# cvg/GeoCalib

Hardware: AMD Instinct MI355X
Metric: images/sec LM calibration (640x480, 20 iters) (higher is better)
Workload: dtype f32

## Files before the change

### geocalib_amd/csrc/gclm_api.hip

```cpp
#include <chrono>
#include <cstdarg>
#include <cstdio>
#include <cstdlib>
#include <cstring>
#include <new>
#include <string>
#include <thread>
#include <vector>

#include "gclm_args.h"
#include "gclm_internal.h"

using namespace gclm;

#ifndef GCLM_FUSED_MAX_WORKGROUPS
#define GCLM_FUSED_MAX_WORKGROUPS 768
#endif
#ifndef GCLM_ROW_PAIRS_DEFAULT
#define GCLM_ROW_PAIRS_DEFAULT -1
#endif
#ifndef GCLM_CONF_PACK_MIN_PIXELS
#define GCLM_CONF_PACK_MIN_PIXELS (256ll << 20)
#endif
#ifndef GCLM_ISO_FINAL
// ... 228 lines not shown
    geo = plan_geometry(B, H, W, aligned16, h->sweep_iters, c.camera_model);
    const bool few = (long long)B * geo.nchunks <= GCLM_FUSED_MAX_WORKGROUPS;
    const bool fusable = !c.shared_intrinsics && geo.vec == 4 && (B == 1 || !c.early_stop) && B > 0 &&
                         !(c.early_stop && h->stop_comm);
    const bool pairable = geo.vec == 4 && five && !(H & 1) && H >= 4 &&
                          (h->row_pairs > 0 ? sweep_has_mirror(c.camera_model) : sweep_mirror_builtin(c.camera_model));
    bool pairs = false;
    if (pairable && h->row_pairs < 0) {
        pairs = !few;
    } else if (pairable && h->row_pairs > 0) {
        pairs = !(h->fused_mode == 1 && fusable);
    }
    one_launch = !pairs && fusable && (h->fused_mode == 1 || (h->fused_mode < 0 && few));
    if (pairs) geo = plan_geometry(B, H, W, aligned16, h->sweep_iters, c.camera_model, true);
}

bool wants_conf_pack(const gclm_handle* h, const Plan& p, bool five, int sweeps, long long pixels) {
    const int model = h->cfg.camera_model;
    return model == GCLM_PINHOLE && p.geo.vec == 4 && five && !p.one_launch && sweeps >= 2 && h->conf_pack != 0 &&
           sweep_has_conf_pack(model) && (h->conf_pack > 0 || (pixels >= GCLM_CONF_PACK_MIN_PIXELS && sweeps >= 6));
}

int make_plan(gclm_handle* h, Plan& p, const Fields& f, int B, int H, int W, const float* sin_lat, int sweeps,
              bool may_pack = true) {
    const int Bp = B > 0 ? B : 1, model = h->cfg.camera_model;
    p = Plan{};
    p.f = f;
    p.choose_walk(h, Bp, H, W, f.aligned16(), f.five());
    SolveCtx& c = h->ctx;
    c.cfg = h->cfg;
    c.B = B; c.H = H; c.W = W; c.nchunks = p.geo.nchunks;
    const bool float4_five = p.geo.vec == 4 && f.five();
    if (sin_lat && float4_five && is_aligned(sin_lat, 16) && (p.one_launch || model != GCLM_PINHOLE)) p.given = sin_lat;
    const bool keep = !p.given && h->slat_plane != 0 && !p.one_launch && float4_five && sweeps >= 2 &&
                      !(h->slat_plane < 0 && model == GCLM_PINHOLE) && sweep_has_slat_plane(model);
    if (int rc = ensure_workspace(h, Bp, p.geo.nchunks, c.n_groups)) return rc;
    p.slat = static_cast<float*>(ensure_plane(h, h->slat, keep ? (size_t)B * H * W * sizeof(float) : 0));
    const long long pixels = (long long)B * H * W;
    const bool pack = may_pack && !p.given && !p.slat && wants_conf_pack(h, p, f.five(), sweeps, pixels);
    p.cpack = static_cast<uint32_t*>(ensure_plane(h, h->cpack, pack ? (size_t)pixels * sizeof(uint32_t) : 0));
    h->cpack_images = p.cpack ? B : 0;
    h->sh.active = false;
    return 0;
}

SweepArgs Plan::next_sweep(const gclm_handle* h, const PBlock* pb, bool loop_params, int stop_step) {
    SweepArgs a{};
    a.up = f.up; a.lat = f.lat; a.upc = f.up ? f.upc : nullptr; a.latc = f.latc;
    a.pb = pb; a.ctrl = h->ctx.ctrl; a.partials = h->ctx.partials;
    a.B = h->ctx.B; a.H = h->ctx.H; a.W = h->ctx.W;
    a.nchunks = geo.nchunks; a.vec = geo.vec;
    a.wu = geo.wu; a.cu = geo.cu; a.nstrips = geo.nstrips; a.rpi = geo.rpi; a.rows_per_block = geo.rows_per_block; a.wpt = geo.wpt; a.jobs = geo.jobs;
    a.hrows = geo.hrows; a.mirror = geo.mirror;
    a.log_focal = loop_params ? h->cfg.use_log_focal : h->ctx.iso_final;
    a.stop_step = stop_step;
    a.up_scale = h->cfg.up_loss_fn_scale; a.lat_scale = h->cfg.lat_loss_fn_scale;
    if (given) {
        a.slat = const_cast<float*>(given);
        a.lat = given;
        a.slat_mode = 2;
    } else if (slat) {
        a.slat = slat;
        if (slat_filled) a.lat = slat;
        a.slat_mode = slat_filled ? 2 : 1;
        slat_filled = true;
    }
    if (cpack) {
        a.cpack = cpack;
        a.cpack_flags = h->ctx.cpack_flags;
        a.cpack_mode = cpack_filled ? 2 : 1;
        cpack_filled = true;
    }
    return a;
}

struct Pacer {
    gclm_handle* h;
    bool paced;
    bool waiting;
    bool stop_seen = false;

    Pacer(gclm_handle* handle, bool single_image_early_stop)
        : h(handle), paced(handle->paced_depth > 0 && single_image_early_stop && handle->progress_host) {
        if (paced && h->paced_cooldown > 0) { --h->paced_cooldown; paced = false; }
        if (paced) h->epoch = (h->epoch + 1) & kPacedEpochMask;
        waiting = paced;
    }
    bool reported(int launch) {
        const unsigned v = __atomic_load_n(h->progress_host, __ATOMIC_ACQUIRE);
        if (((v >> kPacedEpochShift) & kPacedEpochMask) != h->epoch) return false;
        if (v & kPacedStopBit) stop_seen = true;
        return stop_seen || (v & 0xffffu) >= (unsigned)(launch + 1);
    }
    void wait_before(int step) {
        if (!waiting || step < h->paced_depth) return;
        const auto t0 = std::chrono::steady_clock::now();
        for (unsigned spin = 0; !reported(step - h->paced_depth); ++spin) {
            if (spin < 256) continue;
            std::this_thread::yield();
            if ((spin & 0xf) == 0 && std::chrono::steady_clock::now() - t0 > std::chrono::microseconds(kPacedPatienceUs)) {
                waiting = false;
                h->paced_cooldown = kPacedCooldown;
                break;
            }
        }
    }
};

int solve_empty_shard(gclm_handle* h, int H, int W, const InitArgs& ia, hipStream_t s) {
// ... 76 lines not shown
    if (int rc = make_plan(h, p, f, B, H, W, d_sin_lat, h->cfg.num_steps + 1)) return rc;
    if (d_record) {
        p.one_launch = false;
        GCLM_HIP(h, hipMemsetAsync(d_record, 0, sizeof(float) * GCLM_LM_RECORD_STRIDE * (size_t)B * h->cfg.num_steps, s));
        return solve_two_launches_per_step(h, p, ia, d_cam_out, d_grav_out, d_info_out, s, d_record);
    }
    if (p.one_launch) return solve_one_launch_per_step(h, p, ia, d_cam_out, d_grav_out, d_info_out, s);
    return solve_two_launches_per_step(h, p, ia, d_cam_out, d_grav_out, d_info_out, s);
}

}

namespace gclm {
Geometry plan_geometry(int B, int H, int W, bool aligned16, int sweep_iters, int camera_model, bool mirror) {
    Geometry g;
    g.vec = (aligned16 && (W % 4 == 0)) ? 4 : 1;
    g.mirror = (mirror && g.vec == 4 && H % 2 == 0 && H >= 4) ? 1 : 0;
    g.hrows = g.mirror ? H / 2 : H;
    const int rows = g.hrows;
    g.wu = W / g.vec;
    auto waste = [](int used, int lanes) { return (int)(50.0 * (lanes - used) / lanes); };
    if (g.wu <= kMaxTile) {
        g.nstrips = 1;
        g.cu = g.wu;
        g.rpi = 1;
        int best = 1 << 30;
        for (int r = 1; r * g.wu <= kMaxTile; ++r) {
            const int lanes = (r * g.wu + 63) / 64 * 64;
            const int score = waste(r * g.wu, lanes) * 1024 + lanes / 64;
            if (score < best) { best = score; g.rpi = r; }
        }
        g.wpt = (g.rpi * g.wu + 63) / 64;
    } else {
        g.rpi = 1;
        g.cu = 256;
        int best = 1 << 30;
        for (int cu = 128; cu <= kMaxTile; cu += 64) {
            const int ns = (g.wu + cu - 1) / cu;
            const int score = waste(g.wu, ns * cu) * 1024 + cu / 64;
            if (score < best) { best = score; g.cu = cu; }
        }
        g.nstrips = (g.wu + g.cu - 1) / g.cu;
        g.wpt = g.cu / 64;
    }
    int builtin = g.mirror ? 10 : 20;
    if (camera_model != GCLM_PINHOLE && rows % (g.rpi * (g.mirror ? 15 : 30)) == 0) builtin = g.mirror ? 15 : 30;
    int iters = (sweep_iters >= 1 && sweep_iters <= 4096) ? sweep_iters : builtin;
    auto jobs = [&](int it) { return g.nstrips * g.wpt * ((rows + g.rpi * it - 1) / (g.rpi * it)); };
    auto chunks = [&](int it) { return (jobs(it) + kBlock / 64 - 1) / (kBlock / 64); };
    while (iters > 2 && (long long)B * chunks(iters) < 2048) iters = iters > 5 ? iters / 2 : iters - 1;
    g.rows_per_block = g.rpi * iters;
    g.jobs = jobs(iters);
    g.nchunks = chunks(iters);
    return g;
}
}

extern "C" {

int gclm_version(void) { return GCLM_VERSION; }

int gclm_abi_config_size(void) { return (int)sizeof(gclm_config); }

int gclm_default_config(gclm_config* cfg) {
    if (!cfg) return -1;
    std::memset(cfg, 0, sizeof(*cfg));
    cfg->struct_size = (int32_t)sizeof(gclm_config);
    cfg->abi_version = GCLM_VERSION;
    cfg->device = 0;
    cfg->camera_model = GCLM_PINHOLE;
    cfg->num_steps = 30;
    cfg->lambda0 = 0.1f;
    cfg->early_stop = 1;
    cfg->atol = 1e-8f;
    cfg->rtol = 1e-8f;
    cfg->use_spherical_manifold = 1;
    cfg->use_log_focal = 1;
    cfg->up_loss_fn_scale = 1e-2f;
    cfg->lat_loss_fn_scale = 1e-2f;
    cfg->estimate_gravity = cfg->estimate_focal = cfg->estimate_dist = 1;
    cfg->compute_uncertainty = 1;
    return 0;
}

int gclm_create(gclm_handle** out, const gclm_config* cfg) {
    if (!out || !cfg) return fail(nullptr, -1, "gclm_create: null argument");
    *out = nullptr;
    char abuf[256];
    if (const char* msg = abi_mismatch(cfg, abuf)) return fail(nullptr, -5, "gclm_create: %s", msg);
    if (const char* msg = validate(*cfg)) return fail(nullptr, -2, "gclm_create: %s", msg);
    const int device = cfg->device;
    int ndev = 0;
    if (hipGetDeviceCount(&ndev) != hipSuccess || ndev <= 0)
        return fail(nullptr, -11, "gclm_create: no HIP device visible (the HIP path has no CPU fallback)");
    if (device < 0 || device >= ndev) return fail(nullptr, -2, "gclm_create: device %d out of range (%d devices)", device, ndev);
    gclm_handle* h = new (std::nothrow) gclm_handle();
    if (!h) return fail(nullptr, -12, "gclm_create: out of host memory");
    h->cfg = *cfg;
    h->device = device;
    *out = h;
    return 0;
}

int gclm_configure(gclm_handle* h, const gclm_config* cfg) {
    if (!h || !cfg) return -1;
    char abuf[256];
// ... 375 lines not shown
```

### geocalib_amd/csrc/gclm_internal.h

```cpp
#pragma once
#include <hip/hip_runtime.h>
#include <stdint.h>

#include <type_traits>

#include "../../include/gclm.h"

namespace gclm {

constexpr int kBlock = 256;
constexpr int kMaxTile = 512;
constexpr int kNAcc = 16;
constexpr int kNAccMax = 24;
constexpr int kPBlockFloats = 20;
constexpr int kMaxP = GCLM_MAX_PARAMS;
constexpr int kStateFloats = 16;
constexpr int kMaxCallImages = 65535;

enum Acc { A_CU = 0, A_CL = 1, A_G0 = 2, A_H00 = 6 };
__host__ __device__ constexpr int acc_pm(int camera_model) { return camera_model == GCLM_RADIAL ? 5 : 4; }
__host__ __device__ constexpr int acc_floats(int camera_model) { return camera_model == GCLM_RADIAL ? kNAccMax : kNAcc; }
__host__ __device__ constexpr int acc_h(int pm, int i, int j) {
    return 2 + pm + i * pm - (i * (i - 1)) / 2 + (j - i);
}
__host__ __device__ constexpr int num_dist_params(int camera_model) {
    return camera_model == GCLM_PINHOLE ? 0 : (camera_model == GCLM_RADIAL ? 2 : 1);
}

template <typename F>
hipError_t with_camera_model(int camera_model, F&& f) {
    switch (camera_model) {
        case GCLM_PINHOLE: return f(std::integral_constant<int, GCLM_PINHOLE>{});
        case GCLM_SIMPLE_RADIAL: return f(std::integral_constant<int, GCLM_SIMPLE_RADIAL>{});
        case GCLM_RADIAL: return f(std::integral_constant<int, GCLM_RADIAL>{});
        case GCLM_SIMPLE_DIVISIONAL: return f(std::integral_constant<int, GCLM_SIMPLE_DIVISIONAL>{});
        default: return hipErrorInvalidValue;
    }
}

struct __attribute__((aligned(16))) PBlock {
    float ifx, ify, cx, cy;
    float ga, gb, gc, k1;
    float T00, T01, T10, T11;
    float T20, T21, wfx, wfy;
    float k2, pad0, pad1, pad2;
};
static_assert(sizeof(PBlock) == kPBlockFloats * 4, "PBlock layout");

struct __attribute__((aligned(16))) State {
    float w, h, fx, fy, cx, cy, k1, k2;
    float gx, gy, gz;
    float lambda, prev_cost, fails, init_cu, init_cl;
};
static_assert(sizeof(State) == kStateFloats * 4, "State layout");

struct Ctrl {
    int stopped;
    int final_sel;
    int pad[2];
    int notclose[GCLM_MAX_STEPS + 4];
};

__host__ __device__ inline bool stop_fired_before(const Ctrl* ctrl, int step) {
    return step >= 2 && ctrl->notclose[step - 1] == 0;
}

struct SweepArgs {
    const float* up;
    const float* lat;
    const float* upc;
    const float* latc;
    const PBlock* pb;
    const Ctrl* ctrl;
    float* partials;
    int B, H, W;
    int nchunks;
    int vec;
    int wu, cu, nstrips;
    int rpi, rows_per_block;
    int wpt, jobs;
    int log_focal;
    int stop_step;
    float up_scale, lat_scale;
    float* slat;
    int slat_mode;
    int hrows;
    int mirror;
    uint32_t* cpack;
    unsigned* cpack_flags;
    int cpack_mode;
};

struct Geometry {
    int vec, nchunks;
    int wu, cu, nstrips, rpi, rows_per_block, wpt, jobs;
    int mirror, hrows;
};

struct SolveCtx {
    gclm_config cfg;
    int B, H, W, nchunks;
    int iso_final;
    int n_groups, group_size;
    const int32_t* group_of_frame;
    State* state[2];
    PBlock* pb[2];
    PBlock* pb_final;
    float* partials;
    float* partials2;
    float* frame_sys;
    Ctrl* ctrl;
    unsigned* cpack_flags;
};
struct InitArgs {
    const float* cam;
    const float* grav;
    const float* scales;
    const float* prior_focal;
    const float* prior_gravity;
    const float* prior_dist;
    int prior_dist_cols;
    const float* up;
    const float* lat;
};
struct FusedArgs {
    SolveCtx c;
    int step;
    int is_final;
    const float* partials_in;
    unsigned* progress;
    unsigned epoch;
    InitArgs ia;
    int init_here;
};
constexpr unsigned kPacedStopBit = 1u << 16;
constexpr unsigned kPacedEpochShift = 20, kPacedEpochMask = 0xfffu;
constexpr int kPacedPatienceUs = 2000;
constexpr int kPacedCooldown = 64;
constexpr int kMaxMergeParts = 8;
struct MergeStopArgs {
    const Ctrl* ctrl[kMaxMergeParts];
    float* info[kMaxMergeParts];
    int B[kMaxMergeParts];
    int n, num_steps;
};
constexpr int kMaxUpsampleTensors = 8;
struct UpsampleMulti {
    const float* src[kMaxUpsampleTensors];
    float* dst[kMaxUpsampleTensors];
// ... 108 lines not shown
```

### geocalib_amd/csrc/gclm_pass.hip

```cpp
#include <type_traits>

#include "gclm_internal.h"
#include "gclm_device.h"

#ifndef GCLM_MIN_WAVES
#define GCLM_MIN_WAVES 1
#endif
#ifndef GCLM_DIV_WAVES
#define GCLM_DIV_WAVES 3
#endif
#ifndef GCLM_PINHOLE_WAVES
#define GCLM_PINHOLE_WAVES 6
#endif
#ifndef GCLM_RADIAL_WAVES
#define GCLM_RADIAL_WAVES 3
#endif
#ifndef GCLM_REUSE_TNUV
#define GCLM_REUSE_TNUV 1
#endif
#ifndef GCLM_PINHOLE_LDS
#define GCLM_PINHOLE_LDS 51200
#endif
#ifndef GCLM_CPACK_LDS
#define GCLM_CPACK_LDS 30720
#endif
#ifndef GCLM_DYN_LDS
#define GCLM_DYN_LDS 0
#endif
#ifndef GCLM_LAT_PAIRS
#define GCLM_LAT_PAIRS 1
#endif
#ifndef GCLM_MIRROR_WAVES
#define GCLM_MIRROR_WAVES 2
#endif
#ifndef GCLM_MIRROR_WAVES_RADIAL
#define GCLM_MIRROR_WAVES_RADIAL 3
#endif

#ifndef GCLM_TRACE
#define GCLM_TRACE 0
#endif
#if GCLM_TRACE
__device__ unsigned long long g_gclm_trace[64][16];
#define GCLM_T(step, slot) do { if (threadIdx.x == 0 && blockIdx.x == GCLM_TRACE_WG && blockIdx.y == 0 && (step) < 64) g_gclm_trace[(step)][(slot)] = wall_clock64(); } while (0)
extern "C" int gclm_debug_trace(unsigned long long* out) {
    return hipMemcpyFromSymbol(out, HIP_SYMBOL(g_gclm_trace), sizeof(g_gclm_trace)) == hipSuccess ? 0 : -1;
}
#ifndef GCLM_TRACE_WG
#define GCLM_TRACE_WG 0
#endif
#else
#define GCLM_T(step, slot) do {} while (0)
#endif

namespace gclm {

namespace {

typedef float f2 __attribute__((ext_vector_type(2)));

__device__ __forceinline__ float vfma(float a, float b, float c) { return fmaf(a, b, c); }
__device__ __forceinline__ f2 vfma(f2 a, f2 b, f2 c) { return __builtin_elementwise_fma(a, b, c); }
__device__ __forceinline__ float vrsq(float a) { return __frsqrt_rn(a); }
__device__ __forceinline__ f2 vrsq(f2 a) { return f2{__frsqrt_rn(a.x), __frsqrt_rn(a.y)}; }
__device__ __forceinline__ float vrcp_hw(float a) { return __builtin_amdgcn_rcpf(a); }
__device__ __forceinline__ f2 vrcp_hw(f2 a) { return f2{__builtin_amdgcn_rcpf(a.x), __builtin_amdgcn_rcpf(a.y)}; }
__device__ __forceinline__ float vsqrt_hw(float a) { return __builtin_amdgcn_sqrtf(a); }
__device__ __forceinline__ f2 vsqrt_hw(f2 a) { return f2{__builtin_amdgcn_sqrtf(a.x), __builtin_amdgcn_sqrtf(a.y)}; }
__device__ __forceinline__ float vmax(float a, float b) { return fmaxf(a, b); }
__device__ __forceinline__ f2 vmax(f2 a, f2 b) { return f2{fmaxf(a.x, b.x), fmaxf(a.y, b.y)}; }
__device__ __forceinline__ float vclamp(float a, float lo, float hi) { return fminf(fmaxf(a, lo), hi); }
__device__ __forceinline__ f2 vclamp(f2 a, float lo, float hi) {
    return f2{fminf(fmaxf(a.x, lo), hi), fminf(fmaxf(a.y, lo), hi)};
}
__device__ __forceinline__ float vrsq_min1(float y) {
    return __builtin_amdgcn_fmed3f(__frsqrt_rn(y), 0.0f, 1.0f);
}
// ... 462 lines not shown
        }
    }
}

template <int MODEL, typename F>
__device__ __forceinline__ void lat_pair_accumulate(F (&acc)[Layout<MODEL>::NACC], const PixelShared<MODEL, F>& S, const LatRow<F>& A,
                                                    const LatRow<F>& B) {
    constexpr int PM = Layout<MODEL>::PM, ND = Layout<MODEL>::ND;
    const Radial<F>& R = S.R;
    F f[1 + ND];
    f[0] = -vfma(R.tau1x2, S.r2, R.tau);
#pragma unroll
    for (int j = 0; j < ND; ++j) f[1 + j] = R.dtau[j];
#pragma unroll
    for (int r = 0; r < 2; ++r) {
        const LatRow<F>& L = r == 0 ? A : B;
        const F w0 = L.wgt * L.l0, w1 = L.wgt * L.l1;
        acc[A_G0 + 0] = vfma(w0, L.rl, acc[A_G0 + 0]);
        acc[A_G0 + 1] = vfma(w1, L.rl, acc[A_G0 + 1]);
        acc[acc_h(PM, 0, 0)] = vfma(w0, L.l0, acc[acc_h(PM, 0, 0)]);
        acc[acc_h(PM, 0, 1)] = vfma(w0, L.l1, acc[acc_h(PM, 0, 1)]);
        acc[acc_h(PM, 1, 1)] = vfma(w1, L.l1, acc[acc_h(PM, 1, 1)]);
    }
    const F a1 = A.wgt * A.hu, a2 = B.wgt * B.hu;
    const F sAA = vfma(a2, B.hu, a1 * A.hu), sC = vfma(a2, B.rl, a1 * A.rl);
    const F sB0 = vfma(a2, B.l0, a1 * A.l0), sB1 = vfma(a2, B.l1, a1 * A.l1);
#pragma unroll
    for (int m = 0; m <= ND; ++m) {
        acc[A_G0 + 2 + m] = vfma(sC, f[m], acc[A_G0 + 2 + m]);
        acc[acc_h(PM, 0, 2 + m)] = vfma(sB0, f[m], acc[acc_h(PM, 0, 2 + m)]);
        acc[acc_h(PM, 1, 2 + m)] = vfma(sB1, f[m], acc[acc_h(PM, 1, 2 + m)]);
#pragma unroll
        for (int n = m; n <= ND; ++n) acc[acc_h(PM, 2 + m, 2 + n)] = vfma(sAA, f[m] * f[n], acc[acc_h(PM, 2 + m, 2 + n)]);
    }
}

template <int MODEL, bool HAS_UP, bool LOGF, typename F, int EMIT = 0, int GMODE = 0>
__device__ __forceinline__ void pixel_accumulate(const PBlock& P, const HuberK& hk, F u, F px, float v, F dux, F duy,
                                                 F slat, F cu, F cl, F (&acc)[Layout<MODEL>::NACC],
                                                 [[maybe_unused]] float* j_up = nullptr,
                                                 [[maybe_unused]] float* j_lat = nullptr,
                                                 [[maybe_unused]] bool patch = false) {
    PixelShared<MODEL, F> S;
    pixel_shared<MODEL, LOGF, F, GMODE>(P, u, v, patch, S);
    pixel_stage<MODEL, HAS_UP, LOGF, F, EMIT>(P, hk, S, u, px, v, dux, duy, slat, cu, cl, acc, j_up, j_lat);
}

constexpr int kWaveSumLane = 63;
template <int CTRL, int ROW_MASK>
__device__ __forceinline__ float dpp_add(float v) {
    const int moved = __builtin_amdgcn_update_dpp(0, __builtin_bit_cast(int, v), CTRL, ROW_MASK, 0xF, false);
    return v + __builtin_bit_cast(float, moved);
}
__device__ __forceinline__ float wave_sum(float v) {
    v = dpp_add<0xB1, 0xF>(v);
    v = dpp_add<0x4E, 0xF>(v);
    v = dpp_add<0x141, 0xF>(v);
    v = dpp_add<0x140, 0xF>(v);
    v = dpp_add<0x142, 0xA>(v);
    v = dpp_add<0x143, 0xC>(v);
    return v;
}

template <int VEC>
struct Lane;
template <>
struct Lane<4> {
    using F = f2;
    using V = float4;
    static constexpr int kPairs = 2;
    static __device__ __forceinline__ V ld(const float* base, uint32_t byte_off) {
        typedef float v4 __attribute__((ext_vector_type(4)));
        const v4* p = reinterpret_cast<const v4*>(reinterpret_cast<const char*>(base) + byte_off);
        const v4 t = __builtin_nontemporal_load(p);
        return make_float4(t.x, t.y, t.z, t.w);
    }
    static __device__ __forceinline__ void st(float* base, uint32_t byte_off, const F (&v)[2]) {
        typedef float v4 __attribute__((ext_vector_type(4)));
        __builtin_nontemporal_store(v4{v[0].x, v[0].y, v[1].x, v[1].y},
                                    reinterpret_cast<v4*>(reinterpret_cast<char*>(base) + byte_off));
    }
    typedef uint32_t P __attribute__((ext_vector_type(4)));
    static __device__ __forceinline__ P ldp(const uint32_t* base, uint32_t byte_off) {
        return __builtin_nontemporal_load(reinterpret_cast<const P*>(reinterpret_cast<const char*>(base) + byte_off));
    }
    static __device__ __forceinline__ void stp(uint32_t* base, uint32_t byte_off, P w) {
        __builtin_nontemporal_store(w, reinterpret_cast<P*>(reinterpret_cast<char*>(base) + byte_off));
    }
    static __device__ __forceinline__ F get(const V& v, int k) { return k == 0 ? f2{v.x, v.y} : f2{v.z, v.w}; }
    static __device__ __forceinline__ V ones() { return make_float4(1.f, 1.f, 1.f, 1.f); }
    static __device__ __forceinline__ bool any_zero(F a) { return a.x == 0.f || a.y == 0.f; }
    static __device__ __forceinline__ float max_of(const F (&t)[2]) { return fmaxf(fmaxf(fmaxf(t[0].x, t[0].y), t[1].x), t[1].y); }
    static __device__ __forceinline__ F fold(F a) { return f2{fold_halfpi(a.x), fold_halfpi(a.y)}; }
    static __device__ __forceinline__ F xcoord(int x, int k) {
        const float x0 = (float)(x + 2 * k);
        return f2{x0, x0 + 1.0f};
    }
};
template <>
struct Lane<1> {
    using F = float;
    using V = float;
    using P = uint32_t;
    static constexpr int kPairs = 1;
    static __device__ __forceinline__ V ld(const float* base, uint32_t byte_off) {
        return *reinterpret_cast<const float*>(reinterpret_cast<const char*>(base) + byte_off);
    }
    static __device__ __forceinline__ void st(float* base, uint32_t byte_off, const F (&v)[1]) {
        *reinterpret_cast<float*>(reinterpret_cast<char*>(base) + byte_off) = v[0];
    }
    static __device__ __forceinline__ F get(const V& v, int) { return v; }
    static __device__ __forceinline__ V ones() { return 1.f; }
    static __device__ __forceinline__ bool any_zero(F a) { return a == 0.f; }
    static __device__ __forceinline__ float max_of(const F (&t)[1]) { return t[0]; }
    static __device__ __forceinline__ F fold(F a) { return fold_halfpi(a); }
    static __device__ __forceinline__ F xcoord(int x, int) { return (float)x; }
};

template <int VEC>
struct LaneJob {
    bool live;
    int y, y_end, xu;
    uint32_t off, off_step;
};
template <int VEC>
__device__ __forceinline__ LaneJob<VEC> lane_job(const SweepArgs& a, const int chunk) {
    const int tid = threadIdx.x;
    const int lane = tid & 63, wave = tid >> 6;
    const int job = chunk * (kBlock / 64) + wave;
    const int tile = job / a.wpt, tw = job - tile * a.wpt;
    const int rowblock = tile / a.nstrips, strip = tile - rowblock * a.nstrips;
    const int f = tw * 64 + lane;
    const int tr = f / a.cu, tc = f - tr * a.cu;
    LaneJob<VEC> j;
    j.xu = strip * a.cu + tc;
    j.live = job < a.jobs && tr < a.rpi && j.xu < a.wu;
    j.y_end = min((rowblock + 1) * a.rows_per_block, a.hrows);
    j.y = rowblock * a.rows_per_block + tr;
    j.off = ((uint32_t)j.y * (uint32_t)a.W + (uint32_t)(j.xu * VEC)) * 4u;
    j.off_step = (uint32_t)a.rpi * (uint32_t)a.W * 4u;
    return j;
}

template <int VEC>
struct RowData {
    typename Lane<VEC>::V vux, vuy, vlat, vcu, vcl;
    typename Lane<VEC>::P vpk;
};
template <bool HAS_UP, bool HAS_UPC, bool HAS_LATC, int VEC, int CPACK = 0>
__device__ __forceinline__ RowData<VEC> load_row(const float* upx, const float* upy, const float* lat, const float* upc,
                                                 const float* latc, const uint32_t off,
                                                 [[maybe_unused]] const uint32_t* cpk = nullptr) {
    using L = Lane<VEC>;
    RowData<VEC> r;
    r.vcu = L::ones();
    r.vcl = L::ones();
    if constexpr (HAS_UP) {
        r.vux = L::ld(upx, off);
        r.vuy = L::ld(upy, off);
    }
    r.vlat = L::ld(lat, off);
    if constexpr (CPACK == 2) {
        r.vpk = L::ldp(cpk, off);
    } else {
        if constexpr (HAS_UP && HAS_UPC) r.vcu = L::ld(upc, off);
        if constexpr (HAS_LATC) r.vcl = L::ld(latc, off);
    }
    return r;
}

template <int VEC, int CPACK>
__device__ __forceinline__ void row_conf(const RowData<VEC>& r, typename Lane<VEC>::F (&cu)[Lane<VEC>::kPairs],
                                         typename Lane<VEC>::F (&cl)[Lane<VEC>::kPairs], [[maybe_unused]] uint32_t* cp_out,
                                         [[maybe_unused]] const uint32_t off, [[maybe_unused]] bool* cp_bad) {
    using L = Lane<VEC>;
    if constexpr (CPACK == 0) {
#pragma unroll
        for (int k = 0; k < L::kPairs; ++k) { cu[k] = L::get(r.vcu, k); cl[k] = L::get(r.vcl, k); }
    } else {
        static_assert(VEC == 4, "the packed confidence plane: float4 path only");
        auto decode2 = [](uint32_t qa, uint32_t qb) { return f2{(float)qa, (float)qb} * dev::kConfStep; };
        if constexpr (CPACK == 2) {
            const uint32_t w[4] = {r.vpk.x, r.vpk.y, r.vpk.z, r.vpk.w};
#pragma unroll
            for (int k = 0; k < 2; ++k) {
                cu[k] = decode2(w[2 * k] & 0xffffu, w[2 * k + 1] & 0xffffu);
// ... 97 lines not shown
    }
#endif
}

template <int MODEL, bool HAS_UP, bool LOGF, int VEC, int SLAT, bool SHARE>
__device__ __forceinline__ void row_math_mirror(const PBlock& P, const HuberK& hk, const typename Lane<VEC>::F (&col_u)[Lane<VEC>::kPairs],
                                                const typename Lane<VEC>::F (&col_px)[Lane<VEC>::kPairs], const int y, const int y2,
                                                const RowData<VEC>& r, const RowData<VEC>& rm,
                                                typename Lane<VEC>::F (&acc)[Layout<MODEL>::NACC], const bool col_zero,
                                                const bool div_k_tiny, float* slat_out, const uint32_t off, const uint32_t off2) {
    using L = Lane<VEC>;
    using F = typename L::F;
    F slat[L::kPairs], slat2[L::kPairs];
    row_slat<VEC, SLAT>(r, slat, slat_out, off);
    row_slat<VEC, SLAT>(rm, slat2, slat_out, off2);
    const float v = ((float)y - P.cy) * P.ify;
    const float v2 = SHARE ? -v : ((float)y2 - P.cy) * P.ify;
    constexpr int GM = MODEL == GCLM_SIMPLE_DIVISIONAL ? 1 : 0;
    const bool patch = div_k_tiny || __builtin_amdgcn_ballot_w64(col_zero && (v == 0.f || v2 == 0.f)) != 0;
#pragma unroll
    for (int k = 0; k < L::kPairs; ++k) {
        PixelShared<MODEL, F> S;
        pixel_shared<MODEL, LOGF, F, GM>(P, col_u[k], v, patch, S);
        if constexpr (SHARE && LOGF && GCLM_LAT_PAIRS) {
            pixel_stage<MODEL, HAS_UP, LOGF, F, 0, 1>(P, hk, S, col_u[k], col_px[k], v, L::get(r.vux, k), L::get(r.vuy, k), slat[k],
                                                      L::get(r.vcu, k), L::get(r.vcl, k), acc);
            pixel_stage<MODEL, HAS_UP, LOGF, F, 0, 1>(P, hk, S, col_u[k], col_px[k], v2, L::get(rm.vux, k), L::get(rm.vuy, k), slat2[k],
                                                      L::get(rm.vcu, k), L::get(rm.vcl, k), acc);
            LatRow<F> la, lb;
            pixel_stage<MODEL, HAS_UP, LOGF, F, 3, 2>(P, hk, S, col_u[k], col_px[k], v, L::get(r.vux, k), L::get(r.vuy, k), slat[k],
                                                      L::get(r.vcu, k), L::get(r.vcl, k), acc, nullptr, nullptr, &la);
            pixel_stage<MODEL, HAS_UP, LOGF, F, 3, 2>(P, hk, S, col_u[k], col_px[k], v2, L::get(rm.vux, k), L::get(rm.vuy, k), slat2[k],
                                                      L::get(rm.vcu, k), L::get(rm.vcl, k), acc, nullptr, nullptr, &lb);
            lat_pair_accumulate<MODEL, F>(acc, S, la, lb);
        } else {
        pixel_stage<MODEL, HAS_UP, LOGF, F>(P, hk, S, col_u[k], col_px[k], v, L::get(r.vux, k), L::get(r.vuy, k), slat[k],
                                            L::get(r.vcu, k), L::get(r.vcl, k), acc);
        if constexpr (!SHARE) pixel_shared<MODEL, LOGF, F, GM>(P, col_u[k], v2, patch, S);
        pixel_stage<MODEL, HAS_UP, LOGF, F>(P, hk, S, col_u[k], col_px[k], v2, L::get(rm.vux, k), L::get(rm.vuy, k), slat2[k],
                                            L::get(rm.vcu, k), L::get(rm.vcl, k), acc);
        }
    }
}

template <int MODEL, bool HAS_UP, bool HAS_UPC, bool HAS_LATC, bool LOGF, int VEC, int PRE = 0, int SLAT = 0, bool MIRROR = false,
          int CPACK = 0>
__device__ __forceinline__ void sweep_body(const SweepArgs& a, const PBlock& P, const int b, const int chunk,
                                           [[maybe_unused]] const LaneJob<VEC>* pj = nullptr,
                                           [[maybe_unused]] const RowData<VEC>* pre = nullptr) {
    constexpr int NACC = Layout<MODEL>::NACC;
    static_assert(PRE == 0 || SLAT != 1, "the prefetched iterations of the one-launch-per-step kernel store no plane");
    static_assert(CPACK == 0 || (PRE == 0 && !MIRROR && SLAT == 0 && VEC == 4 && HAS_UP && HAS_UPC && HAS_LATC),
                  "the packed confidence plane: the plain five-plane float4 sweep");
    const int tid = threadIdx.x;
    HuberK hk;
    hk.a2u = a.up_scale * a.up_scale;
    hk.inv_a2u = 1.0f / hk.a2u;
    hk.a2l = a.lat_scale * a.lat_scale;
    hk.inv_a2l = 1.0f / hk.a2l;

    const size_t N = (size_t)a.H * a.W;
    const float* upx = HAS_UP ? a.up + (size_t)b * 2 * N : nullptr;
    const float* upy = HAS_UP ? upx + N : nullptr;
    const float* lat = a.lat + (size_t)b * N;
    const float* upc = HAS_UPC ? a.upc + (size_t)b * N : nullptr;
    const float* latc = HAS_LATC ? a.latc + (size_t)b * N : nullptr;
    [[maybe_unused]] float* slat_out = SLAT == 1 ? a.slat + (size_t)b * N : nullptr;
    [[maybe_unused]] uint32_t* cpk = CPACK != 0 ? a.cpack + (size_t)b * N : nullptr;
    [[maybe_unused]] bool cp_bad = false;

    using L = Lane<VEC>;
    using F = typename L::F;
    F acc[NACC];
#pragma unroll
    for (int i = 0; i < NACC; ++i) acc[i] = F(0.f);

    const int lane = tid & 63, wave = tid >> 6;
    const LaneJob<VEC> j = PRE > 0 ? *pj : lane_job<VEC>(a, chunk);
    const int xu = j.xu;
    const bool live = j.live;
    const int y_end = j.y_end;
    int y = j.y;
    uint32_t off = j.off;
    const uint32_t off_step = j.off_step;
    F col_u[L::kPairs], col_px[L::kPairs];
#pragma unroll
    for (int k = 0; k < L::kPairs; ++k) {
        col_u[k] = (L::xcoord(xu * VEC, k) - P.cx) * P.ifx;
        col_px[k] = vfma(col_u[k], vsplat(col_u[k], -P.gc), vsplat(col_u[k], P.ga));
    }
    [[maybe_unused]] bool col_zero = false;
    [[maybe_unused]] const bool div_k_tiny = !(fabsf(P.k1) >= 1e-20f);
    if constexpr (MODEL == GCLM_SIMPLE_DIVISIONAL) {
#pragma unroll
        for (int k = 0; k < L::kPairs; ++k) col_zero = col_zero || L::any_zero(col_u[k]);
    }
    if (live) {
        if constexpr (PRE > 0) {
#pragma unroll
            for (int it = 0; it < PRE; ++it) {
                if (y < y_end) {
                    row_math<MODEL, HAS_UP, LOGF, VEC, SLAT>(P, hk, col_u, col_px, y, pre[it], acc, col_zero, div_k_tiny);
                    y += a.rpi;
                    off += off_step;
                }
            }
        }
        if constexpr (MIRROR) {
            static_assert(PRE == 0 && VEC == 4 && HAS_UP && HAS_UPC && HAS_LATC, "row pairs: five-plane float4 sweep");
            const bool centered = P.cy + P.cy == (float)a.H;
            const uint32_t row_bytes = (uint32_t)a.W * 4u, col_bytes = (uint32_t)(xu * VEC) * 4u;
            auto pair = [&](auto share) {
                const int y2 = y == 0 ? (a.H >> 1) : a.H - y;
                const uint32_t off2 = (uint32_t)y2 * row_bytes + col_bytes;
                const RowData<VEC> r = load_row<HAS_UP, HAS_UPC, HAS_LATC, VEC>(upx, upy, lat, upc, latc, off);
                const RowData<VEC> rm = load_row<HAS_UP, HAS_UPC, HAS_LATC, VEC>(upx, upy, lat, upc, latc, off2);
                __builtin_amdgcn_sched_barrier(0);
                row_math_mirror<MODEL, HAS_UP, LOGF, VEC, SLAT, decltype(share)::value>(P, hk, col_u, col_px, y, y2, r, rm, acc, col_zero,
                                                                                    div_k_tiny, slat_out, off, off2);
                y += a.rpi;
                off += off_step;
            };
            if (centered) {
                if (__builtin_amdgcn_ballot_w64(y == 0) != 0 && y < y_end) pair(std::false_type{});
                while (y < y_end) pair(std::true_type{});
            } else {
                while (y < y_end) pair(std::false_type{});
            }
        } else
        for (; y < y_end; y += a.rpi, off += off_step) {
            const RowData<VEC> r = load_row<HAS_UP, HAS_UPC, HAS_LATC, VEC, CPACK>(upx, upy, lat, upc, latc, off, cpk);
            __builtin_amdgcn_sched_barrier(0);
            row_math<MODEL, HAS_UP, LOGF, VEC, SLAT, CPACK>(P, hk, col_u, col_px, y, r, acc, col_zero, div_k_tiny, slat_out, off,
                                                            cpk, &cp_bad);
        }
        if constexpr (CPACK == 1) { if (cp_bad) atomicOr(a.cpack_flags + b, 1u); }
    }

    __shared__ float red[kBlock / 64][NACC];
    float wsum[NACC];
#pragma unroll
    for (int i = 0; i < NACC; ++i) wsum[i] = wave_sum(hsum(acc[i]));
    if (lane == kWaveSumLane) {
#pragma unroll
        for (int i = 0; i < NACC; ++i) red[wave][i] = wsum[i];
    }
    __syncthreads();
    if (tid < NACC) {
        float s = 0.f;
#pragma unroll
        for (int w = 0; w < kBlock / 64; ++w) s += red[w][tid];
        if (tid == A_CU) s *= hk.a2u;
        if (tid == A_CL) s *= hk.a2l;
        a.partials[((size_t)b * a.nchunks + chunk) * NACC + tid] = s;
    }
}

template <int MODEL, bool HAS_UP, bool HAS_UPC, bool HAS_LATC, bool LOGF, int VEC, int SLAT = 0, bool MIRROR = false>
__global__ __launch_bounds__(kBlock, MIRROR ? (MODEL == GCLM_RADIAL && LOGF ? GCLM_MIRROR_WAVES_RADIAL : GCLM_MIRROR_WAVES) : (VEC == 4 && MODEL == GCLM_RADIAL) ? GCLM_RADIAL_WAVES : (VEC == 4 && MODEL > GCLM_RADIAL) ? GCLM_DIV_WAVES : (VEC == 4 && MODEL == GCLM_SIMPLE_RADIAL) ? 4 : (VEC == 4 && MODEL == GCLM_PINHOLE && LOGF) ? (SLAT == 0 ? GCLM_PINHOLE_WAVES : 5) : GCLM_MIN_WAVES) void sweep_kernel(
    const SweepArgs a) {
    if (stop_fired_before(a.ctrl, a.stop_step)) return;
    const int b = blockIdx.y, chunk = blockIdx.x;
    const PBlock P = a.pb[b];
    sweep_body<MODEL, HAS_UP, HAS_UPC, HAS_LATC, LOGF, VEC, 0, SLAT, MIRROR>(a, P, b, chunk);
}

template <bool LOGF, int CPACK>
__global__ __launch_bounds__(kBlock, 5) void conf_pack_sweep_kernel(const SweepArgs a) {
    if (stop_fired_before(a.ctrl, a.stop_step)) return;
    const int b = blockIdx.y, chunk = blockIdx.x;
    const PBlock P = a.pb[b];
    if constexpr (CPACK == 2) {
        if (a.cpack_flags[b] != 0) {
            sweep_body<GCLM_PINHOLE, true, true, true, LOGF, 4, 0, 0, false, 0>(a, P, b, chunk);
            return;
        }
    }
    sweep_body<GCLM_PINHOLE, true, true, true, LOGF, 4, 0, 0, false, CPACK>(a, P, b, chunk);
}

template <int MODEL, bool HAS_UP, bool HAS_UPC, bool HAS_LATC, bool LOGF, int SLAT = 0>
__global__ __launch_bounds__(kBlock) void fused_step_kernel(const SweepArgs a, const FusedArgs f) {
    using namespace dev;
    constexpr int PM = Layout<MODEL>::PM, NACC = Layout<MODEL>::NACC;
    const SolveCtx& c = f.c;
    const gclm_config& cfg = c.cfg;
    static_assert(SLAT == 0 || (SLAT == 2 && HAS_UP && HAS_UPC && HAS_LATC), "a handed plane: five-plane launches only");
    const int b = blockIdx.y, chunk = blockIdx.x, step = f.step;
    GCLM_T(step, 0);
    __shared__ PBlock Ps;
    __shared__ int go;
    int stop_j = 0;
    if (cfg.early_stop) {
        if (!f.is_final) {
            if (step >= 3 && c.ctrl->notclose[step - 2] == 0) return;
        } else {
            const int lane = threadIdx.x & 63;
            for (int j0 = 1; j0 <= step - 2 && stop_j == 0; j0 += 64) {
                const int j = j0 + lane;
                const int v = j <= step - 2 ? c.ctrl->notclose[j] : 1;
                const unsigned long long m = __builtin_amdgcn_ballot_w64(v == 0);
                if (m) stop_j = j0 + __builtin_ctzll(m);
            }
        }
    }
    constexpr int kFusedPre = 2;
    const LaneJob<4> pj = lane_job<4>(a, chunk);
    RowData<4> pre[kFusedPre];
    auto request_fields = [&]() {
        const size_t N = (size_t)a.H * a.W;
        const float* upx = HAS_UP ? a.up + (size_t)b * 2 * N : nullptr;
        const float* upy = HAS_UP ? upx + N : nullptr;
// ... 209 lines not shown
    if (weight) weight[i] = isx * c;
    if (second) second[i] = y <= 1.0f ? 0.f : -isx / (2.0f * y * a2);
}

constexpr bool sweep_exists(int model, bool up, bool upc, bool latc, bool logf, int vec, int slat, bool mirror, int cpack = 0) {
    const bool five = up && upc && latc;
    if (model < GCLM_PINHOLE || model > GCLM_SIMPLE_DIVISIONAL || (upc && !up) || slat < 0 || slat > 2) return false;
    if (cpack != 0) return (cpack == 1 || cpack == 2) && model == GCLM_PINHOLE && five && vec == 4 && slat == 0 && !mirror;
    if (vec != 4) return vec == 1 && !logf && slat == 0 && !mirror;
    if (mirror) return five && (model == GCLM_RADIAL || model == GCLM_SIMPLE_DIVISIONAL);
    return slat == 0 || five;
}
constexpr bool fused_exists(int model, bool up, bool upc, bool latc, int slat) {
    if (model < GCLM_PINHOLE || model > GCLM_SIMPLE_DIVISIONAL || (upc && !up)) return false;
    return slat == 0 || (slat == 2 && up && upc && latc);
}
constexpr int kMirrorBuiltinModels = (1 << GCLM_RADIAL) | (1 << GCLM_SIMPLE_DIVISIONAL);

template <typename F>
hipError_t with_flags(F&& f) { return f(); }
template <typename F, typename... Bools>
hipError_t with_flags(F&& f, bool first, Bools... rest) {
    auto bind = [&](auto c) { return with_flags([&](auto... cs) { return f(c, cs...); }, rest...); };
    return first ? bind(std::true_type{}) : bind(std::false_type{});
}
template <typename F>
hipError_t with_slat_mode(int slat_mode, F&& f) {
    switch (slat_mode) {
        case 0: return f(std::integral_constant<int, 0>{});
        case 1: return f(std::integral_constant<int, 1>{});
        case 2: return f(std::integral_constant<int, 2>{});
        default: return hipErrorInvalidValue;
    }
}

}

hipError_t launch_sweep(int camera_model, const SweepArgs& a, hipStream_t s) {
    if (a.B <= 0) return hipSuccess;
    if ((a.slat_mode != 0 && a.slat == nullptr) || (a.mirror != 0 && ((a.H & 1) || a.hrows * 2 != a.H))) return hipErrorInvalidValue;
    if (a.cpack_mode != 0 && (a.cpack == nullptr || a.cpack_flags == nullptr)) return hipErrorInvalidValue;
    const dim3 grid(a.nchunks, a.B), block(kBlock);
    const bool up = a.up != nullptr, vec4 = a.vec == 4;
    return with_camera_model(camera_model, [&](auto m) {
        return with_slat_mode(a.slat_mode, [&](auto sl) {
          return with_slat_mode(a.cpack_mode, [&](auto cp) {
            return with_flags([&](auto u, auto uc, auto lc, auto lf, auto v4, auto mir) {
                constexpr int MODEL = decltype(m)::value, SLAT = decltype(sl)::value, VEC = decltype(v4)::value ? 4 : 1;
                constexpr int CPACK = decltype(cp)::value;
                constexpr bool U = decltype(u)::value, UC = decltype(uc)::value, LC = decltype(lc)::value,
                               LOGF = decltype(lf)::value, MIRROR = decltype(mir)::value;
                if constexpr (sweep_exists(MODEL, U, UC, LC, LOGF, VEC, SLAT, MIRROR, CPACK)) {
                    constexpr unsigned lds = (MODEL == GCLM_PINHOLE && VEC == 4 && SLAT == 0 && !MIRROR && GCLM_DYN_LDS == 0)
                                                 ? (CPACK == 2 ? GCLM_CPACK_LDS : GCLM_PINHOLE_LDS) : GCLM_DYN_LDS;
                    if constexpr (CPACK != 0) hipLaunchKernelGGL((conf_pack_sweep_kernel<LOGF, CPACK>), grid, block, lds, s, a);
                    else hipLaunchKernelGGL((sweep_kernel<MODEL, U, UC, LC, LOGF, VEC, SLAT, MIRROR>), grid, block, lds, s, a);
                    return hipGetLastError();
                } else {
                    return hipErrorInvalidValue;
                }
            }, up, up && a.upc != nullptr, a.latc != nullptr, vec4 && a.log_focal != 0, vec4, a.mirror != 0);
          });
        });
    });
}

bool sweep_has_mirror(int camera_model) { return sweep_exists(camera_model, true, true, true, true, 4, 0, true); }
bool sweep_mirror_builtin(int camera_model) { return sweep_has_mirror(camera_model) && ((kMirrorBuiltinModels >> camera_model) & 1) != 0; }
bool sweep_has_slat_plane(int camera_model) { return sweep_exists(camera_model, true, true, true, true, 4, 1, false); }
bool sweep_has_conf_pack(int camera_model) { return sweep_exists(camera_model, true, true, true, true, 4, 0, false, 1); }

hipError_t launch_fused_step(int camera_model, const SweepArgs& a, const FusedArgs& f, hipStream_t s) {
    if (a.B <= 0) return hipSuccess;
    if (a.vec != 4 || (a.slat_mode != 0 && (a.slat == nullptr || a.lat != a.slat))) return hipErrorInvalidValue;
    const dim3 grid(a.nchunks, a.B), block(kBlock);
    const bool up = a.up != nullptr;
    return with_camera_model(camera_model, [&](auto m) {
        return with_slat_mode(a.slat_mode, [&](auto sl) {
            return with_flags([&](auto u, auto uc, auto lc, auto lf) {
                constexpr int MODEL = decltype(m)::value, SLAT = decltype(sl)::value;
                constexpr bool U = decltype(u)::value, UC = decltype(uc)::value, LC = decltype(lc)::value, LOGF = decltype(lf)::value;
                if constexpr (fused_exists(MODEL, U, UC, LC, SLAT)) {
                    hipLaunchKernelGGL((fused_step_kernel<MODEL, U, UC, LC, LOGF, SLAT>), grid, block, 0, s, a, f);
                    return hipGetLastError();
                } else {
                    return hipErrorInvalidValue;
                }
            }, up, up && a.upc != nullptr, a.latc != nullptr, a.log_focal != 0);
        });
    });
}

hipError_t launch_residual_fields(int camera_model, const float* d_up, const float* d_lat, const float* d_cam,
                                  const float* d_grav, int B, int H, int W, float* d_r_up, float* d_r_lat, hipStream_t s) {
    if (B <= 0 || H <= 0 || W <= 0) return hipSuccess;
    const dim3 grid((unsigned)(((size_t)H * W + kBlock - 1) / kBlock), B), block(kBlock);
    return with_camera_model(camera_model, [&](auto m) {
        hipLaunchKernelGGL(residual_kernel<decltype(m)::value>, grid, block, 0, s, d_up, d_lat, d_cam, d_grav, H, W, d_r_up, d_r_lat);
        return hipGetLastError();
    });
}

hipError_t launch_huber_costs(const float* d_residual, size_t n, int dim, float scale, const float* d_conf,
                              float* d_cost, float* d_weight, float* d_second, hipStream_t s) {
    if (n == 0) return hipSuccess;
    hipLaunchKernelGGL(huber_costs_kernel, dim3((unsigned)((n + 255) / 256)), dim3(256), 0, s, d_residual, n, dim, scale,
                       d_conf, d_cost, d_weight, d_second);
// ... 16 lines not shown
```

Before: 58920.

## Precompute divisors and Huber constants on host, batch DPP wave reductions

Replaces the integer divisions in lane job mapping with host-precomputed magic-multiply reciprocals, and passes the Huber scale constants in the kernel arguments instead of recomputing them per thread. It also makes the wave index scalar via readfirstlane, reduces only the live accumulators with row-broadcast DPP steps batched eight at a time in inline asm, and changes the LDS and launch-bounds settings for some variants. The goal is fewer VALU instructions in setup and the reduction epilogue, at the cost of hand-written asm hazards (s_nop) and subtle range limits on the fast division.

Measured after the change: 59140 (median of 6 runs). Within noise of the previous version (+0.4%).

```diff
diff --git a/geocalib_amd/csrc/gclm_api.hip b/geocalib_amd/csrc/gclm_api.hip
--- a/geocalib_amd/csrc/gclm_api.hip
+++ b/geocalib_amd/csrc/gclm_api.hip
@@ -304,9 +304,12 @@
     a.nchunks = geo.nchunks; a.vec = geo.vec;
     a.wu = geo.wu; a.cu = geo.cu; a.nstrips = geo.nstrips; a.rpi = geo.rpi; a.rows_per_block = geo.rows_per_block; a.wpt = geo.wpt; a.jobs = geo.jobs;
     a.hrows = geo.hrows; a.mirror = geo.mirror;
+    a.div_wpt = geo.div_wpt; a.div_nstrips = geo.div_nstrips; a.div_cu = geo.div_cu;
     a.log_focal = loop_params ? h->cfg.use_log_focal : h->ctx.iso_final;
     a.stop_step = stop_step;
     a.up_scale = h->cfg.up_loss_fn_scale; a.lat_scale = h->cfg.lat_loss_fn_scale;
+    a.a2u = a.up_scale * a.up_scale; a.inv_a2u = 1.0f / a.a2u;
+    a.a2l = a.lat_scale * a.lat_scale; a.inv_a2l = 1.0f / a.a2l;
     if (given) {
         a.slat = const_cast<float*>(given);
         a.lat = given;
@@ -489,6 +492,9 @@
     g.rows_per_block = g.rpi * iters;
     g.jobs = jobs(iters);
     g.nchunks = chunks(iters);
+    g.div_wpt = div_u31_make((uint32_t)g.wpt);
+    g.div_nstrips = div_u31_make((uint32_t)g.nstrips);
+    g.div_cu = div_u16_make((uint32_t)g.cu);
     return g;
 }
 }
diff --git a/geocalib_amd/csrc/gclm_geom.h b/geocalib_amd/csrc/gclm_geom.h
--- /dev/null
+++ b/geocalib_amd/csrc/gclm_geom.h
@@ -0,0 +1,39 @@
+#pragma once
+#include <stdint.h>
+
+#if defined(__HIPCC__) || defined(__CUDACC__)
+#define GCLM_HD __host__ __device__
+#else
+#define GCLM_HD
+#endif
+
+namespace gclm {
+
+struct DivU31 {
+    uint32_t mul, shift;
+};
+GCLM_HD inline DivU31 div_u31_make(uint32_t d) {
+    uint32_t l = 0;
+    while (l < 31 && (1u << l) < d) ++l;
+    const uint64_t p = (uint64_t)1 << (31 + l);
+    return DivU31{(uint32_t)((p + d - 1) / d), 31 + l};
+}
+GCLM_HD inline uint32_t div_u31(uint32_t n, DivU31 k) { return (uint32_t)(((uint64_t)n * k.mul) >> k.shift); }
+
+struct DivU16 {
+    uint32_t hi, lo;
+};
+constexpr uint32_t kDivU16MaxDividend = 1u << 16, kDivU16MaxDivisor = 2048;
+GCLM_HD inline DivU16 div_u16_make(uint32_t d) {
+    const uint32_t m = ((1u << 27) + d - 1) / d;
+    return DivU16{m >> 12, m & 0xfffu};
+}
+GCLM_HD inline uint32_t div_u16(uint32_t f, DivU16 k) {
+#if defined(__HIP_DEVICE_COMPILE__)
+    return (__umul24(f, k.hi) + (__umul24(f, k.lo) >> 12)) >> 15;
+#else
+    return (f * k.hi + ((f * k.lo) >> 12)) >> 15;
+#endif
+}
+
+}
diff --git a/geocalib_amd/csrc/gclm_internal.h b/geocalib_amd/csrc/gclm_internal.h
--- a/geocalib_amd/csrc/gclm_internal.h
+++ b/geocalib_amd/csrc/gclm_internal.h
@@ -5,6 +5,7 @@
 #include <type_traits>
 
 #include "../../include/gclm.h"
+#include "gclm_geom.h"
 
 namespace gclm {
 
@@ -79,9 +80,12 @@
     int wu, cu, nstrips;
     int rpi, rows_per_block;
     int wpt, jobs;
+    DivU31 div_wpt, div_nstrips;
+    DivU16 div_cu;
     int log_focal;
     int stop_step;
     float up_scale, lat_scale;
+    float a2u, inv_a2u, a2l, inv_a2l;
     float* slat;
     int slat_mode;
     int hrows;
@@ -95,6 +99,8 @@
     int vec, nchunks;
     int wu, cu, nstrips, rpi, rows_per_block, wpt, jobs;
     int mirror, hrows;
+    DivU31 div_wpt, div_nstrips;
+    DivU16 div_cu;
 };
 
 struct SolveCtx {
diff --git a/geocalib_amd/csrc/gclm_pass.hip b/geocalib_amd/csrc/gclm_pass.hip
--- a/geocalib_amd/csrc/gclm_pass.hip
+++ b/geocalib_amd/csrc/gclm_pass.hip
@@ -23,6 +23,9 @@
 #endif
 #ifndef GCLM_CPACK_LDS
 #define GCLM_CPACK_LDS 30720
+#endif
+#ifndef GCLM_CPACK_FILL_LDS
+#define GCLM_CPACK_FILL_LDS GCLM_PINHOLE_LDS
 #endif
 #ifndef GCLM_DYN_LDS
 #define GCLM_DYN_LDS 0
@@ -591,14 +594,50 @@
     const int moved = __builtin_amdgcn_update_dpp(0, __builtin_bit_cast(int, v), CTRL, ROW_MASK, 0xF, false);
     return v + __builtin_bit_cast(float, moved);
 }
-__device__ __forceinline__ float wave_sum(float v) {
+__device__ __forceinline__ float row_sum(float v) {
     v = dpp_add<0xB1, 0xF>(v);
     v = dpp_add<0x4E, 0xF>(v);
     v = dpp_add<0x141, 0xF>(v);
     v = dpp_add<0x140, 0xF>(v);
-    v = dpp_add<0x142, 0xA>(v);
-    v = dpp_add<0x143, 0xC>(v);
     return v;
+}
+__device__ __forceinline__ void rows_sum8(float (&v)[8]) {
+#define GCLM_DPP8(ctl) \
+    "v_add_f32_dpp %0, %0, %0 " ctl "\n\tv_add_f32_dpp %1, %1, %1 " ctl "\n\tv_add_f32_dpp %2, %2, %2 " ctl "\n\t" \
+    "v_add_f32_dpp %3, %3, %3 " ctl "\n\tv_add_f32_dpp %4, %4, %4 " ctl "\n\tv_add_f32_dpp %5, %5, %5 " ctl "\n\t" \
+    "v_add_f32_dpp %6, %6, %6 " ctl "\n\tv_add_f32_dpp %7, %7, %7 " ctl "\n\t"
+    asm("s_nop 1\n\t" GCLM_DPP8("row_bcast:15 row_mask:0xa bank_mask:0xf") GCLM_DPP8("row_bcast:31 row_mask:0xc bank_mask:0xf")
+        : "+v"(v[0]), "+v"(v[1]), "+v"(v[2]), "+v"(v[3]), "+v"(v[4]), "+v"(v[5]), "+v"(v[6]), "+v"(v[7]));
+#undef GCLM_DPP8
+}
+template <int MODEL>
+constexpr bool acc_live(int idx) {
+    constexpr int PM = Layout<MODEL>::PM, PN = Layout<MODEL>::PN;
+    if (idx == A_CU || idx == A_CL) return true;
+    for (int i = 0; i < PN; ++i) {
+        if (idx == A_G0 + i) return true;
+        for (int j = i; j < PN; ++j)
+            if (idx == acc_h(PM, i, j)) return true;
+    }
+    return false;
+}
+template <int MODEL>
+__device__ __forceinline__ void wave_sum(float (&v)[Layout<MODEL>::NACC]) {
+    constexpr int NACC = Layout<MODEL>::NACC;
+    struct Live { int n, idx[NACC]; };
+    constexpr Live live = [] { Live l{}; for (int i = 0; i < NACC; ++i) if (acc_live<MODEL>(i)) l.idx[l.n++] = i; return l; }();
+    constexpr int NL = live.n;
+#pragma unroll
+    for (int g = 0; g < NL; g += 8) {
+        float t[8];
+#pragma unroll
+        for (int i = 0; i < 8; ++i) t[i] = g + i < NL ? row_sum(v[live.idx[g + i < NL ? g + i : 0]]) : t[NL - 1 - g];
+        rows_sum8(t);
+#pragma unroll
+        for (int i = 0; i < 8; ++i) if (g + i < NL) v[live.idx[g + i]] = t[i];
+    }
+#pragma unroll
+    for (int i = 0; i < NACC; ++i) if (!acc_live<MODEL>(i)) v[i] = 0.f;
 }
 
 template <int VEC>
@@ -662,15 +701,15 @@
     int y, y_end, xu;
     uint32_t off, off_step;
 };
-template <int VEC>
+template <int VEC, bool UNIFORM = true>
 __device__ __forceinline__ LaneJob<VEC> lane_job(const SweepArgs& a, const int chunk) {
     const int tid = threadIdx.x;
-    const int lane = tid & 63, wave = tid >> 6;
+    const int lane = tid & 63, wave = UNIFORM ? __builtin_amdgcn_readfirstlane(tid >> 6) : (tid >> 6);
     const int job = chunk * (kBlock / 64) + wave;
-    const int tile = job / a.wpt, tw = job - tile * a.wpt;
-    const int rowblock = tile / a.nstrips, strip = tile - rowblock * a.nstrips;
+    const int tile = (int)div_u31((uint32_t)job, a.div_wpt), tw = job - tile * a.wpt;
+    const int rowblock = (int)div_u31((uint32_t)tile, a.div_nstrips), strip = tile - rowblock * a.nstrips;
     const int f = tw * 64 + lane;
-    const int tr = f / a.cu, tc = f - tr * a.cu;
+    const int tr = (int)div_u16((uint32_t)f, a.div_cu), tc = f - (int)__umul24((uint32_t)tr, (uint32_t)a.cu);
     LaneJob<VEC> j;
     j.xu = strip * a.cu + tc;
     j.live = job < a.jobs && tr < a.rpi && j.xu < a.wu;
@@ -874,12 +913,13 @@
     static_assert(PRE == 0 || SLAT != 1, "the prefetched iterations of the one-launch-per-step kernel store no plane");
     static_assert(CPACK == 0 || (PRE == 0 && !MIRROR && SLAT == 0 && VEC == 4 && HAS_UP && HAS_UPC && HAS_LATC),
                   "the packed confidence plane: the plain five-plane float4 sweep");
-    const int tid = threadIdx.x;
-    HuberK hk;
-    hk.a2u = a.up_scale * a.up_scale;
-    hk.inv_a2u = 1.0f / hk.a2u;
-    hk.a2l = a.lat_scale * a.lat_scale;
-    hk.inv_a2l = 1.0f / hk.a2l;
+    constexpr bool kScalarSetup = !(MIRROR && !LOGF);
+    const int wave = __builtin_amdgcn_readfirstlane((int)threadIdx.x >> 6);
+    HuberK hk{a.inv_a2u, a.a2u, a.inv_a2l, a.a2l};
+    if constexpr (!kScalarSetup) {
+        hk.a2u = a.up_scale * a.up_scale; hk.inv_a2u = 1.0f / hk.a2u;
+        hk.a2l = a.lat_scale * a.lat_scale; hk.inv_a2l = 1.0f / hk.a2l;
+    }
 
     const size_t N = (size_t)a.H * a.W;
     const float* upx = HAS_UP ? a.up + (size_t)b * 2 * N : nullptr;
@@ -897,8 +937,7 @@
 #pragma unroll
     for (int i = 0; i < NACC; ++i) acc[i] = F(0.f);
 
-    const int lane = tid & 63, wave = tid >> 6;
-    const LaneJob<VEC> j = PRE > 0 ? *pj : lane_job<VEC>(a, chunk);
+    const LaneJob<VEC> j = PRE > 0 ? *pj : lane_job<VEC, kScalarSetup>(a, chunk);
     const int xu = j.xu;
     const bool live = j.live;
     const int y_end = j.y_end;
@@ -962,7 +1001,10 @@
     __shared__ float red[kBlock / 64][NACC];
     float wsum[NACC];
 #pragma unroll
-    for (int i = 0; i < NACC; ++i) wsum[i] = wave_sum(hsum(acc[i]));
+    for (int i = 0; i < NACC; ++i) wsum[i] = hsum(acc[i]);
+    wave_sum<MODEL>(wsum);
+    const int lane = kScalarSetup ? (int)__builtin_amdgcn_mbcnt_hi(~0u, __builtin_amdgcn_mbcnt_lo(~0u, 0u)) : (int)(threadIdx.x & 63);
+    const int tid = kScalarSetup ? wave * 64 + lane : (int)threadIdx.x;
     if (lane == kWaveSumLane) {
 #pragma unroll
         for (int i = 0; i < NACC; ++i) red[wave][i] = wsum[i];
@@ -979,7 +1021,7 @@
 }
 
 template <int MODEL, bool HAS_UP, bool HAS_UPC, bool HAS_LATC, bool LOGF, int VEC, int SLAT = 0, bool MIRROR = false>
-__global__ __launch_bounds__(kBlock, MIRROR ? (MODEL == GCLM_RADIAL && LOGF ? GCLM_MIRROR_WAVES_RADIAL : GCLM_MIRROR_WAVES) : (VEC == 4 && MODEL == GCLM_RADIAL) ? GCLM_RADIAL_WAVES : (VEC == 4 && MODEL > GCLM_RADIAL) ? GCLM_DIV_WAVES : (VEC == 4 && MODEL == GCLM_SIMPLE_RADIAL) ? 4 : (VEC == 4 && MODEL == GCLM_PINHOLE && LOGF) ? (SLAT == 0 ? GCLM_PINHOLE_WAVES : 5) : GCLM_MIN_WAVES) void sweep_kernel(
+__global__ __launch_bounds__(kBlock, MIRROR ? (MODEL == GCLM_RADIAL && LOGF ? GCLM_MIRROR_WAVES_RADIAL : GCLM_MIRROR_WAVES) : (VEC == 4 && MODEL == GCLM_RADIAL) ? GCLM_RADIAL_WAVES : (VEC == 4 && MODEL > GCLM_RADIAL) ? GCLM_DIV_WAVES : (VEC == 4 && MODEL == GCLM_SIMPLE_RADIAL) ? 4 : (VEC == 4 && MODEL == GCLM_PINHOLE) ? (LOGF && SLAT == 0 ? GCLM_PINHOLE_WAVES : 5) : GCLM_MIN_WAVES) void sweep_kernel(
     const SweepArgs a) {
     if (stop_fired_before(a.ctrl, a.stop_step)) return;
     const int b = blockIdx.y, chunk = blockIdx.x;
@@ -1295,7 +1337,7 @@
                                LOGF = decltype(lf)::value, MIRROR = decltype(mir)::value;
                 if constexpr (sweep_exists(MODEL, U, UC, LC, LOGF, VEC, SLAT, MIRROR, CPACK)) {
                     constexpr unsigned lds = (MODEL == GCLM_PINHOLE && VEC == 4 && SLAT == 0 && !MIRROR && GCLM_DYN_LDS == 0)
-                                                 ? (CPACK == 2 ? GCLM_CPACK_LDS : GCLM_PINHOLE_LDS) : GCLM_DYN_LDS;
+                                                 ? (CPACK == 2 ? GCLM_CPACK_LDS : CPACK == 1 ? GCLM_CPACK_FILL_LDS : GCLM_PINHOLE_LDS) : GCLM_DYN_LDS;
                     if constexpr (CPACK != 0) hipLaunchKernelGGL((conf_pack_sweep_kernel<LOGF, CPACK>), grid, block, lds, s, a);
                     else hipLaunchKernelGGL((sweep_kernel<MODEL, U, UC, LC, LOGF, VEC, SLAT, MIRROR>), grid, block, lds, s, a);
                     return hipGetLastError();
```
